# lehy/ocaml-hnsw

Measured on AMD Instinct MI355X. Metric: queries/sec at recall@10>=0.95, SIFT1M d=128 ef=128 k=10, higher is better.
Workload: dtype u8

## Files before the change

### include/hnsw_mi355x.h

```cpp
#ifndef HNSW_MI355X_H
#define HNSW_MI355X_H

#include <stdint.h>

#ifdef __cplusplus
extern "C" {
#endif

#define HNSW_ABI_VERSION 3

typedef struct hnsw_index hnsw_index;

enum {
    HNSW_OK = 0,
    HNSW_ERR_BAD_ARG = -1,
    HNSW_ERR_EMPTY_INDEX = -2,
    HNSW_ERR_DEGREE_OVERFLOW = -3,
    HNSW_ERR_NO_DEVICE = -4,
    HNSW_ERR_HIP = -5,
    HNSW_ERR_OOM = -6,
    HNSW_ERR_UNSUPPORTED = -7
};

enum { HNSW_METRIC_L2 = 0,
// ... 53 lines not shown
    int32_t row_format;
} hnsw_index_info;

int32_t hnsw_abi_version(void);
const char *hnsw_last_error(void);
int32_t hnsw_device_count(int32_t *count);

int32_t hnsw_index_create(const hnsw_index_desc *desc, int32_t device, hnsw_index **out);
int32_t hnsw_index_destroy(hnsw_index *idx);
int32_t hnsw_index_get_info(const hnsw_index *idx, hnsw_index_info *info);
int32_t hnsw_index_set_option(hnsw_index *idx, const char *name, int64_t value);
int32_t hnsw_index_row_bytes(const hnsw_index *idx, int64_t *row_bytes);
int32_t hnsw_index_sq8_params(const hnsw_index *idx, float *lo, float *scale);
int32_t hnsw_index_sq8_codes(const hnsw_index *idx, uint8_t *out);
int32_t hnsw_index_kernel_times(hnsw_index *idx, double *search_ms, double *prepass_ms, int32_t *calls);

int32_t hnsw_search_batch(hnsw_index *idx, const float *queries, int64_t nq, int64_t q_stride,
                          const hnsw_search_params *params, int32_t *out_ids, float *out_dist,
                          uint32_t *out_ndist, uint32_t *out_nhops);

int32_t hnsw_host_register(void *p, int64_t bytes);
int32_t hnsw_host_unregister(void *p);
int32_t hnsw_host_alloc(void **out, int64_t bytes);
int32_t hnsw_host_free(void *p);

int32_t hnsw_search_batch_device(hnsw_index *idx, const float *d_queries, int64_t nq,
                                 int64_t q_stride, const hnsw_search_params *params,
                                 int32_t *d_ids, float *d_dist, uint32_t *d_ndist,
                                 uint32_t *d_nhops, uint32_t *d_status, void *stream);

// ... 129 lines not shown
```

### ocaml-hnsw_amd/__init__.py

```python
import ctypes as _C
import os as _os

import numpy as _np

_PKG_DIR = _os.path.dirname(_os.path.abspath(__file__)) if "__file__" in globals() and \
    _os.path.basename(_os.path.dirname(_os.path.abspath(__file__))) == "ocaml-hnsw_amd" else \
    _os.path.join(_os.path.dirname(_os.path.abspath(__file__)), "ocaml-hnsw_amd")
LIB_PATH = _os.environ.get("HNSW_LIB_PATH") or _os.path.join(_PKG_DIR, "libhnsw_mi355x.so")

OK, ERR_BAD_ARG, ERR_EMPTY_INDEX, ERR_DEGREE_OVERFLOW = 0, -1, -2, -3
ERR_NO_DEVICE, ERR_HIP, ERR_OOM, ERR_UNSUPPORTED = -4, -5, -6, -7
METRIC_L2, METRIC_IP = 0, 1
FILL_OHNSW, FILL_BA = 0, 1
SEM_OHNSW, SEM_FUNCTOR, SEM_FUNCTOR_NEAREST_K = 0, 1, 2
ROWS_F32, ROWS_BYTES, ROWS_SPLIT, ROWS_HALF, ROWS_SQ8 = 0, 2, 3, 4, 5

ABI_VERSION = 3

_vp, _i32, _i64, _str, _f32 = _C.c_void_p, _C.c_int32, _C.c_int64, _C.c_char_p, _C.c_float
_ABI = {
    "hnsw_abi_version": (None, _i32),
    "hnsw_last_error": (None, _str),
    "hnsw_device_count": [_vp],
    "hnsw_index_create": [_vp, _i32, _vp],
# ... 27 lines not shown
    "hnsw_index_insert": [_vp, _vp, _i64, _i64, _vp],
    "hnsw_select_neighbours_batch": [_vp, _vp, _i64, _i64, _vp, _vp, _i32, _i32, _i32, _vp, _vp, _vp],
    "hnsw_index_layer_stats": [_vp, _i32, _vp],
    "hnsw_index_layer_isolated": [_vp, _i32, _vp, _i64, _vp],
    "hnsw_index_locality_codes": [_vp, _vp],
    "hnsw_index_visited_blocks": [_vp, _vp, _vp],
    "hnsw_index_prepare": [_vp, _vp],
    "hnsw_index_save": [_vp, _str],
    "hnsw_index_load": [_str, _i32, _vp],
    "hnsw_index_export_layer0": [_vp, _vp, _vp],
    "hnsw_index_export_upper_count": [_vp, _i32, _vp],
    "hnsw_index_export_upper": [_vp, _i32, _vp, _vp, _vp],
    "hnsw_search_layer_batch": [_vp, _i32, _vp, _i64, _i64, _vp, _i32, _vp, _vp, _vp, _vp, _vp, _vp],
    "hnsw_search_one_batch": [_vp, _i32, _vp, _i64, _i64, _vp, _vp, _vp],
    "hnsw_index_kernel_times": [_vp, _vp, _vp, _vp],
    "hnsw_search_submit": [_vp, _vp, _i64, _i64, _vp, _vp],
    "hnsw_search_wait": [_vp, _vp, _vp, _vp, _vp],
    "hnsw_multi_create": [_vp, _vp, _i32, _vp],
    "hnsw_multi_destroy": [_vp],
    "hnsw_multi_num_replicas": [_vp, _vp],
    "hnsw_multi_replica": [_vp, _i32, _vp],
    "hnsw_multi_search_batch": [_vp, _vp, _i64, _i64, _vp, _vp, _vp, _vp, _vp],
    "hnsw_multi_search_batch_device": [_vp, _vp, _i64, _i64, _vp, _vp, _vp],
    "hnsw_multi_copy_result": [_vp, _i32, _vp, _vp],
    "hnsw_multi_debug_counters": [_vp, _vp],
    "hnsw_host_register": [_vp, _i64],
    "hnsw_host_unregister": [_vp],
    "hnsw_host_alloc": [_vp, _i64],
    "hnsw_host_free": [_vp],
}
# ... 301 lines not shown
        return _np.float32(lo.value), _np.float32(s.value)

    def sq8_codes(self):
        out = _np.empty((self.info().n, self.d), _np.uint8)
        _check(load().hnsw_index_sq8_codes(self.handle, _ptr(out)))
        return out

    def filter(self, allow):
        return Filter(self, allow)

    def kernel_times(self):
        s_, p_, n_ = _C.c_double(0), _C.c_double(0), _C.c_int32(0)
        _check(load().hnsw_index_kernel_times(self.handle, _C.byref(s_), _C.byref(p_), _C.byref(n_)))
        return s_.value, p_.value, n_.value

    def release(self):
        if self._index is not None:
            load().hnsw_index_destroy(self._index)
            self._index = None

    def __del__(self):
        try:
            self.release()
        except Exception:
            pass


class _HostBlock:

    def __init__(self, shape, dtype):
# ... 453 lines not shown
```

### ocaml-hnsw_amd/build.py

```python
#!/usr/bin/env python3
import os
import subprocess
import sys

HERE = os.path.dirname(os.path.abspath(__file__))
CSRC = os.path.join(HERE, "csrc")
ROOT = os.path.dirname(HERE)
LIB = os.path.join(HERE, "libhnsw_mi355x.so")
SOURCES = ["hnsw_capi.hip", "hnsw_build.hip", "hnsw_layer_ops.hip", "hnsw_multi.hip", "hnsw_order.hip", "hnsw_rows8.hip",
           "hnsw_rows_split.hip", "hnsw_rows16.hip", "hnsw_rows_sq8.hip", "hnsw_locality.hip", "hnsw_scan.hip", "hnsw_rerank.hip", "hnsw_filter.hip",
           "hnsw_range.hip"]
VARIANT_SOURCE = "hnsw_search_variants.hip"
VARIANTS = [(m, s, f) for m in (0, 1) for s in (0, 1) for f in (0, 1, 2, 3, 4)]
DEPS = SOURCES + [VARIANT_SOURCE, "hnsw_device.hip.h", "hnsw_hop_asm.hip.h", "hnsw_hop_loop.inc", "hnsw_hop_slots.inc", "hnsw_hop_instances.inc", "hnsw_scan_slab.inc", "hnsw_build_device.hip.h", "hnsw_internal.h",
        os.path.join(ROOT, "include", "hnsw_mi355x.h")]


def _hipcc():
    for c in (os.environ.get("HIPCC"), "/opt/rocm/bin/hipcc", "hipcc"):
        if c and (os.path.isabs(c) and os.path.exists(c) or not os.path.isabs(c)):
            return c
    return "hipcc"


def up_to_date():
    if not os.path.exists(LIB):
        return False
    t = os.path.getmtime(LIB)
    for d in DEPS + [os.path.abspath(__file__)]:
# ... 88 lines not shown
```

### ocaml-hnsw_amd/csrc/hnsw_capi.hip

```cpp
#include "hnsw_internal.h"

#include <mutex>

using hnsw_dev::IndexView;
using hnsw_dev::SearchArgs;
using namespace hnsw_host;

__global__ void __launch_bounds__(64)
probe_queries_kernel(const IndexView iv, int64_t step, float *out) {
    const int64_t v = (int64_t)blockIdx.x * step;
    const int32_t nb = iv.nbr0[v * iv.S0];
    const int64_t u = nb >= 0 ? (int64_t)nb : v;
    for (int64_t i = threadIdx.x; i < iv.stride; i += 64)
        out[(int64_t)blockIdx.x * iv.stride + i] = 0.5f * (iv.X[v * iv.stride + i] + iv.X[u * iv.stride + i]);
}

__global__ void __launch_bounds__(1024)
flagged_list_kernel(const uint32_t *status, int64_t nq, int32_t *map, int32_t cap) {
    __shared__ int32_t count;
    if (threadIdx.x == 0) count = 0;
    for (int i = threadIdx.x; i < cap; i += blockDim.x) map[i] = -1;
    __syncthreads();
    for (int64_t q = threadIdx.x; q < nq; q += blockDim.x)
        if (status[q] & 1u) { const int at = atomicAdd(&count, 1); if (at < cap) map[at] = (int32_t)q; }
// ... 377 lines not shown
    if (nq == 0) return HNSW_OK;
    if (!buffers) return fail(HNSW_ERR_BAD_ARG, "null buffer");
    if (q_stride < idx->iv.d) return fail(HNSW_ERR_BAD_ARG, "q_stride < d");
    return HNSW_OK;
}

int launch_rerun(hnsw_index *idx, const hnsw_search_params &p, const KnnBatch &b, const int32_t *qmap, int64_t c, uint32_t *slab,
                 int32_t cap, hipStream_t st) {
    const KnnShape sh = knn_shape(idx, p.ef, p.semantics);
    SearchArgs a = knn_args(p, b, knn_vt_bits(idx, sh), knn_blk_bits(idx, sh));
    a.nq = c; a.qmap = qmap; a.q_limit = b.nq; a.ovf_g = slab; a.ovf_gcap = cap;
    a.any_flag = nullptr;
    return launch_search_args(idx, sh, a, st);
}

int knn_search(hnsw_index *idx, const hnsw_search_params *caller_params, const KnnBatch &caller_b, hipStream_t st, float *d_stage,
               RefineBufs *walk, bool raw_walk) {
    int rc = check_batch(idx, caller_params, caller_b.nq, caller_b.q_stride, caller_b.Q && caller_b.ids && caller_b.dist);
    if (rc || caller_b.nq == 0) return rc;
    HIP_TRY(hipSetDevice(idx->device));
    const int refine_c = raw_walk ? 0 : refine_count(idx, caller_params);
    hnsw_search_params walk_params = *caller_params;
    KnnBatch b = caller_b;
    if (refine_c > 0) {
        walk_params.k = refine_c;
        if ((rc = refine_walk(caller_b, refine_c, walk ? *walk : idx->refine_scratch, &b))) return rc;
    }
    const hnsw_search_params *params = &walk_params;
    const KnnShape sh = knn_shape(idx, params->ef, params->semantics);
    void *block = nullptr;
    Event *ev = nullptr;
    if (idx->time_kernels && idx->tev_used + 3 <= 3 * 4096) {
        while (idx->tev.size() < idx->tev_used + 3) {
            Event e;
            HIP_TRY(hipEventCreate(&e.h));
            idx->tev.push_back(std::move(e));
        }
        ev = &idx->tev[idx->tev_used];
        HIP_TRY(hipEventRecord(ev[0], st));
    }
    const bool sq8 = idx->info.row_format == HNSW_ROWS_SQ8;
    const float *rerank_Q = nullptr;
    if (sq8) {
        if ((rc = sq8_walk_queries(idx, walk ? *walk : idx->refine_scratch, &b, true, d_stage, st))) return rc;
        rerank_Q = d_stage ? d_stage : caller_b.Q;
        d_stage = nullptr;
    }
    SearchArgs a = knn_args(*params, b, knn_vt_bits(idx, sh), knn_blk_bits(idx, sh));
    const int mode = idx->order_mode;
    if (mode != 0 && (mode == 1 || 2 * b.nq > resident_queries(idx, sh).queries)) {
        rc = order_longest_first(idx, b.Q, b.nq, b.q_stride, d_stage, st, &block, &a.qmap, &a.pre_entry, &a.pre_key, &a.pre_nd, &a.pre_layer);
        if (rc) return rc;
// ... 51 lines not shown
}

hipError_t knn_download(const KnnBatch &b, int k, int32_t *ids, float *dist, uint32_t *nd, uint32_t *nh, hipStream_t st) {
    const size_t rbytes = (size_t)b.nq * k * 4, cbytes = (size_t)b.nq * 4;
    hipError_t e = hipSuccess;
    if (ids) e = hipMemcpyAsync(ids, b.ids, rbytes, hipMemcpyDeviceToHost, st);
    if (dist && e == hipSuccess) e = hipMemcpyAsync(dist, b.dist, rbytes, hipMemcpyDeviceToHost, st);
    if (nd && e == hipSuccess) e = hipMemcpyAsync(nd, b.nd, cbytes, hipMemcpyDeviceToHost, st);
    if (nh && e == hipSuccess) e = hipMemcpyAsync(nh, b.nh, cbytes, hipMemcpyDeviceToHost, st);
    return e;
}

int ensure_host_call_state(hnsw_index *idx) {
    if (!idx->hs[0]) HIP_TRY(hipStreamCreateWithFlags(&idx->hs[0].h, hipStreamNonBlocking));
    if (!idx->hFlag) {
        HIP_TRY(idx->hFlag.alloc(64, hipHostMallocMapped));
        HIP_TRY(hipHostGetDevicePointer((void **)&idx->hFlagDev, idx->hFlag, 0));
    }
    return HNSW_OK;
}

int HostInput::resolve(const void *p, size_t n, DevBuf &stage) {
    bytes = n; from = nullptr;
    if ((dev = registered_device_address(p, n))) return HNSW_OK;
    const int rc = stage.ensure(n);
    dev = stage.p; from = p;
    return rc;
}
int HostInput::upload(hipStream_t st) const {
    if (from) HIP_TRY(hipMemcpyAsync(const_cast<void *>(dev), from, bytes, hipMemcpyHostToDevice, st));
    return HNSW_OK;
}
// ... 24 lines not shown
        if (out_nd) znd = (uint32_t *)(s + 3 * SMALL_BLOCK);
        if (out_nh) znh = (uint32_t *)(s + 4 * SMALL_BLOCK);
    }
    k = k_;
    b = idx->scratch.batch(nq, q_stride, k);
    b.Q = (const float *)q.dev;
    if (zi) b.ids = zi, b.dist = zd;
    if (znd) b.nd = znd;
    if (znh) b.nh = znh;
    ids = zi && !small ? nullptr : out_ids; dist = zi && !small ? nullptr : out_dist;
    nd = znd && !small ? nullptr : out_nd; nh = znh && !small ? nullptr : out_nh;
    if (q_in_place) *q_in_place = !q.from;
    return q.upload(idx->hs[0]);
}

int HostCall::finish(hnsw_index *idx, const char *what, hipStream_t st) {
    const hipError_t ed = small ? hipSuccess : knn_download(b, k, ids, dist, nd, nh, st), es = st ? hipStreamSynchronize(st) : hipDeviceSynchronize();
    if (ed != hipSuccess) return hip_fail(ed, "result download");
    if (es != hipSuccess) return fail(HNSW_ERR_HIP, "%s failed: %s", what, hipGetErrorString(es));
    if (small) {
        const size_t rbytes = (size_t)b.nq * k * 4, cbytes = (size_t)b.nq * 4;
        memcpy(ids, idx->hSmall + SMALL_BLOCK, rbytes); memcpy(dist, idx->hSmall + 2 * SMALL_BLOCK, rbytes);
        if (nd) memcpy(nd, idx->hSmall + 3 * SMALL_BLOCK, cbytes);
        if (nh) memcpy(nh, idx->hSmall + 4 * SMALL_BLOCK, cbytes);
    }
    return HNSW_OK;
}

int trial_search(hnsw_index *idx, hnsw_search_params p) {
    int rc = ensure_host_call_state(idx);
    if (rc) return rc;
    DevBuf out;
// ... 295 lines not shown
                HIP_TRY(hipSetDevice(idx->device));
                HIP_TRY(hipDeviceSynchronize());
                idx->tables.Xq.release();
            }
            idx->sq8_on = false;
        }
        bind_view(idx);
        idx->forget_shapes();
        return HNSW_OK;
    }
    if (!strcmp(name, "refine")) {
        if (value < -1 || value > 1024) return fail(HNSW_ERR_BAD_ARG, "refine=%lld: 0 (off), 1..1024 candidates or -1 (all of W)", (long long)value);
        idx->refine = (int)value;
        return HNSW_OK;
    }
    if (!strcmp(name, "time_kernels")) { idx->time_kernels = value != 0; return HNSW_OK; }
    if (!strcmp(name, "visited_blocks")) {
        idx->blk_mode = value < 0 ? -1 : (value ? 1 : 0);
        idx->forget_shapes();
        return HNSW_OK;
    }
    if (!strcmp(name, "device_fallback_slab_bytes")) {
        HIP_TRY(hipSetDevice(idx->device));
        HIP_TRY(hipDeviceSynchronize());
        idx->dFbSlab.release(); idx->dFbMap.release(); idx->fb_queries = 0;
        if (value <= 0) return HNSW_OK;
        const int64_t per_query = std::max<int64_t>(idx->iv.n, 1) * 4;
        const int64_t q = std::min<int64_t>(value / per_query, 65536);
        if (q < 1) return fail(HNSW_ERR_BAD_ARG, "device_fallback_slab_bytes=%lld holds no query: one needs 4 n = %lld bytes", (long long)value, (long long)per_query);
        int rc;
        DevBuf slab, map;
// ... 21 lines not shown
    for (size_t i = 0; i < n; ++i) {
        float a = 0, b = 0;
        HIP_TRY(hipEventSynchronize(idx->tev[3 * i + 2]));
        HIP_TRY(hipEventElapsedTime(&a, idx->tev[3 * i], idx->tev[3 * i + 1]));
        HIP_TRY(hipEventElapsedTime(&b, idx->tev[3 * i + 1], idx->tev[3 * i + 2]));
        if (idx->tev_ordered[i]) p += a;
        s += b;
    }
    idx->tev_used = 0;
    if (search_ms) *search_ms = n ? s / (double)n : 0.0;
    if (prepass_ms) *prepass_ms = n ? p / (double)n : 0.0;
    if (calls) *calls = (int32_t)n;
    return HNSW_OK;
}

int32_t hnsw_search_batch(hnsw_index *idx, const float *queries, int64_t nq, int64_t q_stride,
                          const hnsw_search_params *params, int32_t *out_ids, float *out_dist,
                          uint32_t *out_ndist, uint32_t *out_nhops) {
    int rc = check_batch(idx, params, nq, q_stride, queries && out_ids && out_dist);
    if (rc || nq == 0) return rc;
    HIP_TRY(hipSetDevice(idx->device));
    HostCall c;
    bool q_in_place = false;
    if ((rc = c.begin(idx, queries, nq, q_stride, params->k, out_ids, out_dist, out_ndist, out_nhops, true, &q_in_place))) return rc;
    hipStream_t st = idx->hs[0];
    c.b.any_flag = idx->hFlagDev;
    *(volatile uint32_t *)idx->hFlag = 0;
    rc = knn_search(idx, params, c.b, st, q_in_place ? (float *)idx->scratch.q.p : nullptr);
    if (rc) { (void)hipStreamSynchronize(st); return rc; }
    if ((rc = c.finish(idx, "search", st))) return rc;
    if (*(volatile uint32_t *)idx->hFlag & 1u) {
        if ((rc = knn_repair(idx, params, c.b, nullptr))) return rc;
        return c.finish(idx, "result download", nullptr);
    }
    return HNSW_OK;
}

int32_t hnsw_search_batch_h2d(hnsw_index *idx, const float *queries, int64_t nq, int64_t q_stride,
                              const hnsw_search_params *params, int32_t *d_ids, float *d_dist,
                              uint32_t *d_ndist, uint32_t *d_nhops, uint32_t *d_status, void *stream) {
    int rc = check_batch(idx, params, nq, q_stride, queries && d_ids && d_dist);
    if (rc || nq == 0) return rc;
    HIP_TRY(hipSetDevice(idx->device));
    const size_t qbytes = query_bytes(nq, q_stride, idx->iv.d);
    if ((rc = idx->scratch.q.ensure(qbytes))) return rc;
    hipStream_t st = (hipStream_t)stream;
// ... 196 lines not shown
```

### ocaml-hnsw_amd/csrc/hnsw_device.hip.h

```cpp
#pragma once

#include <hip/hip_runtime.h>
#include <stdint.h>

namespace hnsw_dev {

constexpr uint32_t KEY_INF = 0xFFFFFFFFu;

struct IndexView {
    const float *X;
    int64_t stride;
    int64_t n;
    int32_t d;
    int32_t nchunks;
    const int32_t *nbr0;
    int32_t S0;
    int32_t SU;
    const int32_t *nbrU;
    int64_t rowsU;
    const int32_t *upper_off;
    const uint8_t *upper_lvl;
    const int2 *upper_ref;
    int32_t max_layer;
    int32_t entry_point;
    int32_t id_base;
    union { const uint8_t *X8; const uint2 *Xh; };
    int32_t stride8;
    const float *Xm;
    const float *tail0;
    int32_t stride_m;
    int32_t main_chunks;
    int32_t tail_chunks;
    const int32_t *lcode;
    const int32_t *lcode0;
};

struct SearchArgs {
    const float *Q;
    int64_t q_stride;
    int64_t nq;
    int32_t ef, k, fill;
    int32_t sem;
    int32_t vt_bits;
    int32_t blk_bits;
    int32_t lds_pad;
    int32_t *out_ids;
    float *out_dist;
    uint32_t *out_ndist, *out_nhops, *out_status;
    const int32_t *qmap;
    int64_t q_limit;
// ... 1029 lines not shown
        }
        cx.qint = ballot(ok) == ~0ull;
        cx.q2 = reduce16_i32((int32_t)sq);
    }
}
template <int NCH>
__device__ __forceinline__ void load_row(float4 (&qv)[NCH], const IndexView &iv, int node, int l16) {
    const float4 *row = reinterpret_cast<const float4 *>(iv.X) + (int64_t)node * (iv.stride >> 2);
#pragma unroll
    for (int i = 0; i < NCH; ++i) {
        const int c = i * 16 + l16;
        qv[i] = (c < iv.nchunks) ? row[c] : make_float4(0.f, 0.f, 0.f, 0.f);
    }
}

constexpr int search_min_waves(int NCH, int NSLOT, int METRIC, int ROWS) {
    return (NCH <= 2 && NSLOT <= 2 && METRIC == 0 && ROWS == 1) ? 7 : (NCH == 2 && NSLOT <= 4 && METRIC == 0 && ROWS == 2) ? 8 : 1;
}
template <int NCH, int RB, int NSLOT, int METRIC, int SEMF, int ROWS, int BLK = 0>
__global__ void __launch_bounds__(64, search_min_waves(NCH, NSLOT, METRIC, ROWS))
hnsw_search_kernel(const IndexView iv, const SearchArgs a) {
    extern __shared__ uint32_t lds[];
    const int lane = threadIdx.x;
    if ((int64_t)blockIdx.x >= a.nq) return;
    const int64_t q = a.qmap ? a.qmap[blockIdx.x] : (int64_t)blockIdx.x;
    if (a.q_limit && (q < 0 || q >= a.q_limit)) return;
    WaveCtx cx = make_ctx(lds, a.vt_bits, lane, BLK ? a.blk_bits : 0);
    if (a.ovf_g) { cx.ovf.g = a.ovf_g + (int64_t)blockIdx.x * a.ovf_gcap; cx.ovf.gcap = a.ovf_gcap; }
    if constexpr (NSLOT >= 3 || (NSLOT == 2 && ROWS != 2)) visited_three_ways(cx, iv.n);
    if ((int)blockIdx.x < a.prio_head || (int)blockIdx.x >= a.prio_tail) __builtin_amdgcn_s_setprio(3);
// ... 33 lines not shown
    search_layer<NCH, RB, NSLOT, METRIC, SEMF, ROWS, BLK>(iv, qv, 0, w, a.ef | (a.lds_pad << 16), cx, n_dist, n_hops, status);
#else
    search_layer<NCH, RB, NSLOT, METRIC, SEMF, ROWS, BLK>(iv, qv, 0, w, a.ef, cx, n_dist, n_hops, status);
#endif

    int wbase = NSLOT * 64 - a.ef;
    if (a.sem == 2) { const int cnt = wlist_count(w); wbase += cnt > a.k ? cnt - a.k : 0; }
#pragma unroll
    for (int s = 0; s < NSLOT; ++s) {
        const int idx = s * 64 + lane - wbase;
        if (idx >= 0 && idx < a.k) {
            int32_t oid = -1;
            float od = a.fill == 0 ? __uint_as_float(0x7FC00000u) : __uint_as_float(0x7F800000u);
            const uint32_t hi = w.hi[s];
            if (hi < DUMMY_HI) { oid = (int32_t)key_id(w.lo[s]) + iv.id_base; od = key_to_dist<METRIC>(hi); }
            a.out_ids[q * a.k + idx] = oid;
            a.out_dist[q * a.k + idx] = od;
        }
    }
    if (lane == 0) {
#ifdef HNSW_TIMING
        if (a.out_ndist) a.out_ndist[q] = (uint32_t)t_start__;
        if (a.out_nhops) a.out_nhops[q] = (uint32_t)wall_clock64();
#else
        if (a.out_ndist) a.out_ndist[q] = n_dist;
        if (a.out_nhops) a.out_nhops[q] = n_hops;
#endif
        if (a.out_status) a.out_status[q] = status;
#ifndef HNSW_PHASE_TIMING
        if ((status & 1u) && a.any_flag) *reinterpret_cast<volatile uint32_t *>(a.any_flag) = 1u;
#endif
    }
}

template <int NCH, int RB, int METRIC, int ROWS = -1>
__global__ void __launch_bounds__(64)
hnsw_descent_kernel(const IndexView iv, const float *Q, int64_t q_stride, int64_t nq, int32_t to_layer,
                    int32_t *out_entry, uint32_t *out_key, uint32_t *out_nd,
                    uint32_t *out_sortkey, int32_t *out_index, float *stage) {
    extern __shared__ uint32_t lds[];
    const int lane = threadIdx.x;
    const int64_t q = blockIdx.x;
    if (q >= nq) return;
    WaveCtx cx = make_ctx(lds, 4, lane);
    float4 qv[NCH];
    load_query<NCH>(qv, Q + q * q_stride, iv.d, cx.l16);
// ... 103 lines not shown
```

### ocaml-hnsw_amd/csrc/hnsw_internal.h

```cpp
#pragma once
#include "../../include/hnsw_mi355x.h"
#include "hnsw_device.hip.h"

#include <algorithm>
#include <cmath>
#include <cstdarg>
#include <cstdio>
#include <cstdlib>
#include <cstring>
#include <memory>
#include <string>
#include <type_traits>
#include <vector>

namespace hnsw_host {


constexpr int RB_NCH2 = 4;
constexpr int rows_in_flight(int nch, bool compact = false) {
    return nch == 1 ? 8 : nch == 2 ? RB_NCH2 : nch == 4 ? (compact ? 4 : 2) : nch == 8 ? (compact ? 2 : 1) : 1;
}
constexpr bool has_odd_nslot(int nch) { return nch == 2 || nch == 4; }

template <int V> using Int = std::integral_constant<int, V>;
// ... 103 lines not shown
    const float *Q;
    int64_t nq, q_stride;
    int32_t *ids;
    float *dist;
    uint32_t *nd, *nh, *st, *any_flag;
};

inline size_t query_bytes(int64_t nq, int64_t q_stride, int d) { return ((size_t)(nq - 1) * q_stride + d) * sizeof(float); }

struct BatchBufs {
    DevBuf q, ids, dist, nd, nh, st, flag, scan;
    KnnBatch batch(int64_t nq, int64_t q_stride, int k, int64_t row0 = 0) const {
        return {(const float *)q.p, nq, q_stride, (int32_t *)ids.p + row0 * k, (float *)dist.p + row0 * k,
                (uint32_t *)nd.p, (uint32_t *)nh.p, (uint32_t *)st.p, (uint32_t *)flag.p};
    }
    int ensure(int64_t nq, size_t qbytes, int k) {
        int rc;
        if ((rc = q.ensure(qbytes)) || (rc = ids.ensure((size_t)nq * k * 4)) || (rc = dist.ensure((size_t)nq * k * 4)) ||
            (rc = nd.ensure((size_t)nq * 4)) || (rc = nh.ensure((size_t)nq * 4)) || (rc = st.ensure((size_t)nq * 4)) || (rc = flag.ensure(16)))
            return rc;
        return HNSW_OK;
    }
    void release() { for (DevBuf *b : {&q, &ids, &dist, &nd, &nh, &st, &flag, &scan}) b->release(); }
};

struct RefineBufs {
    DevBuf ids, dist, nd, qt;
    int ensure(int64_t nq, int c) {
        int rc;
        if ((rc = ids.ensure((size_t)nq * c * 4)) || (rc = dist.ensure((size_t)nq * c * 4)) || (rc = nd.ensure((size_t)nq * 4))) return rc;
        return HNSW_OK;
    }
};

struct FilterBufs {
    DevBuf wids, wdist, wnd, wnh, wst;
// ... 65 lines not shown
    int lcode_state = 0;
    int blk_mode = -1;
    struct ShapeChoice {
        int blk = -1;
        int vt_bits = 0;
        int per_cu = -1;
        size_t lds = 0;
    } shape[hnsw_host::SLOT_CLASSES][2];
    void forget_shapes(bool keep_visited = false) {
        for (auto &c : shape) for (ShapeChoice &s : c) s = ShapeChoice{keep_visited ? s.blk : -1};
    }
    int cus = 0;
    hnsw_host::BatchBufs scratch;
    hnsw_host::Pinned<uint32_t> hFlag;
    uint32_t *hFlagDev = nullptr;
    hnsw_host::Pinned<char> hSmall;
    char *hSmallDev = nullptr;
    hnsw_host::DevBuf dFbSlab, dFbMap;
    int64_t fb_queries = 0;
    hnsw_host::Stream hs[4];
    std::vector<hnsw_request *> free_requests;
    std::vector<std::unique_ptr<hnsw_request>> all_requests;
    int live_requests = 0, next_stream = 0;
    bool time_kernels = false;
    std::vector<hnsw_host::Event> tev;
    size_t tev_used = 0;
    std::vector<char> tev_ordered;
    struct OrderScratch { hipStream_t st; hnsw_host::Table block; };
    std::vector<OrderScratch> order_scratch;
    int order_mode = -1;
    int vt_bits_override = 0;
    int lds_pad = -1;
    int scan_slabs = 0;
    std::vector<std::pair<int, int>> prepared;
    bool byte_rows_off = false, split_rows_off = false, split_rows_freed = false;
    bool half_rows_on = false;
    int refine = 0;
    hnsw_host::RefineBufs refine_scratch;
    bool sq8_on = false;
    float sq8_lo = 0.0f, sq8_scale = 1.0f;
    hnsw_host::FilterBufs filter_scratch;
    hnsw_host::RangeBufs range_scratch;
// ... 55 lines not shown
struct HostInput {
    const void *dev = nullptr, *from = nullptr;
    size_t bytes = 0;
    int resolve(const void *p, size_t n, DevBuf &stage);
    int upload(hipStream_t st) const;
};
struct HostCall {
    KnnBatch b{};
    int k = 0;
    bool small = false;
    int32_t *ids = nullptr;
    float *dist = nullptr;
    uint32_t *nd = nullptr, *nh = nullptr;
    int begin(::hnsw_index *idx, const float *queries, int64_t nq, int64_t q_stride, int k, int32_t *out_ids, float *out_dist,
              uint32_t *out_nd, uint32_t *out_nh, bool allow_small, bool *q_in_place = nullptr);
    int finish(::hnsw_index *idx, const char *what, hipStream_t st);
};

inline int search_vt_bits(const hnsw_index *idx, int ef) {
    int b = idx->vt_bits_override;
    if (b <= 0) {
        b = ef <= 256 ? 11 : 12;
    }
    b = std::max(4, std::min(16, b));
    while (b < 16 && ((int64_t)0xFFFF << (b - 1)) < idx->iv.n) ++b;
    return b;
}

template <class Launch>
int rerun_overflowed(hnsw_index *idx, int64_t nq, const uint32_t *d_status, Launch &&launch) {
    std::vector<uint32_t> st((size_t)nq);
// ... 20 lines not shown
```

### ocaml-hnsw_amd/csrc/hnsw_multi.hip

```cpp
#include "hnsw_internal.h"

#include <dlfcn.h>
#include <rccl/rccl.h>

using namespace hnsw_host;

namespace {

struct RcclApi {
    void *lib = nullptr;
    ncclResult_t (*CommInitAll)(ncclComm_t *, int, const int *) = nullptr;
    ncclResult_t (*CommDestroy)(ncclComm_t) = nullptr;
    ncclResult_t (*CommAbort)(ncclComm_t) = nullptr;
    ncclResult_t (*AllGather)(const void *, void *, size_t, ncclDataType_t, ncclComm_t, hipStream_t) = nullptr;
    ncclResult_t (*Broadcast)(const void *, void *, size_t, ncclDataType_t, int, ncclComm_t, hipStream_t) = nullptr;
    ncclResult_t (*GroupStart)() = nullptr;
    ncclResult_t (*GroupEnd)() = nullptr;
    const char *(*GetErrorString)(ncclResult_t) = nullptr;
};

int load_rccl(RcclApi &api) {
    if (api.lib) return HNSW_OK;
    void *h = nullptr;
    for (const char *name : {"librccl.so.1", "librccl.so", "/opt/rocm/lib/librccl.so.1"}) {
// ... 84 lines not shown
}

int search_and_gather(hnsw_multi *m, const float *queries, int64_t nq, int64_t q_stride, const hnsw_search_params *params,
                      uint32_t *out_ndist, uint32_t *out_nhops) {
    const int G = (int)m->replicas.size();
    const int k = params->k;
    int rc;
    if ((rc = ensure_streams(m)) || (rc = ensure_comms(m))) return rc;
    const int d = m->replicas[0]->iv.d;
    const size_t full = (size_t)nq * k;
    for (int g = 0; g < G; ++g) {
        const int64_t lo = shard_lo(nq, g, G), hi = shard_lo(nq, g + 1, G);
        hnsw_index *idx = m->replicas[(size_t)g];
        BatchBufs &b = m->buf[(size_t)g];
        HIP_TRY(hipSetDevice(m->devices[(size_t)g]));
        if ((rc = b.ids.ensure(std::max<size_t>(full, 1) * 4)) || (rc = b.dist.ensure(std::max<size_t>(full, 1) * 4)) || (rc = b.flag.ensure(16)))
            return rc;
        m->hFlags[g] = 0;
        if (hi <= lo) continue;
        const int64_t ns = hi - lo;
        const size_t qbytes = query_bytes(ns, q_stride, d);
        if ((rc = b.q.ensure(qbytes)) || (rc = b.nd.ensure((size_t)ns * 4)) || (rc = b.nh.ensure((size_t)ns * 4)) || (rc = b.st.ensure((size_t)ns * 4)))
            return rc;
        hipStream_t st = m->streams[(size_t)g];
        const KnnBatch shard = b.batch(ns, q_stride, k, lo);
        HIP_TRY(hipMemsetAsync(shard.any_flag, 0, 4, st));
        HIP_TRY(hipMemcpyAsync(b.q.p, queries + lo * q_stride, qbytes, hipMemcpyHostToDevice, st));
        if ((rc = knn_search(idx, params, shard, st))) return rc;
        HIP_TRY(hipMemcpyAsync(&m->hFlags[g], shard.any_flag, 4, hipMemcpyDeviceToHost, st));
    }
    auto exchange = [&](int only_shard) -> int {
// ... 195 lines not shown
```

### ocaml-hnsw_amd/csrc/hnsw_order.hip

```cpp
#include "hnsw_internal.h"

#include <hipcub/hipcub.hpp>

using hnsw_dev::IndexView;
using namespace hnsw_host;

namespace {
constexpr int ORDER_BUCKETS = 2048;
constexpr int ORDER_THREADS = 1024;
template <int PER>
__global__ void __launch_bounds__(ORDER_THREADS)
order_bucket_kernel(const uint32_t *sortkey, int32_t n, int32_t *order) {
    __shared__ uint32_t cnt[ORDER_BUCKETS];
    __shared__ uint32_t red_min[ORDER_THREADS / 64], red_max[ORDER_THREADS / 64];
    __shared__ uint32_t part[ORDER_THREADS];
    const int t = threadIdx.x;
    uint32_t keys[PER > 0 ? PER : 1];
    uint32_t lo = 0xFFFFFFFFu, hi = 0u;
    if (PER > 0) {
#pragma unroll
        for (int j = 0; j < PER; ++j) { const int i = t + j * ORDER_THREADS; keys[j] = sortkey[i < n ? i : 0]; }
#pragma unroll
        for (int j = 0; j < PER; ++j) if (t + j * ORDER_THREADS < n) { lo = keys[j] < lo ? keys[j] : lo; hi = keys[j] > hi ? keys[j] : hi; }
    } else {
// ... 70 lines not shown
    uint32_t *key = d_scratch, *nd = d_scratch + nq, *sortkey = d_scratch + 2 * nq;
    int32_t *index = (int32_t *)(d_scratch + 3 * nq);
    const int rows = idx->info.row_format == HNSW_ROWS_BYTES ? HNSW_ROWS_BYTES : HNSW_ROWS_F32;
    const hipError_t e = launch_descent(idx, rows, d_queries, q_stride, nq, to_layer, d_entry, key, nd, sortkey, index, nullptr, st);
    if (e != hipSuccess) return fail(HNSW_ERR_HIP, "descent launch failed: %s", hipGetErrorString(e));
    return HNSW_OK;
}

int order_longest_first(::hnsw_index *idx, const float *d_queries, int64_t nq, int64_t q_stride, float *d_stage, hipStream_t st,
                        void **block, const int32_t **qmap, const int32_t **pre_entry, const uint32_t **pre_key,
                        const uint32_t **pre_nd, int32_t *pre_layer) {
    const int32_t to_layer = 1;
    *pre_layer = to_layer;
    *block = nullptr;
    const size_t n = (size_t)nq, slot = (n * 4 + 255) & ~(size_t)255;
    size_t temp_bytes = 0;
    if (hipcub::DeviceRadixSort::SortPairs(nullptr, temp_bytes, (const uint32_t *)nullptr, (uint32_t *)nullptr,
                                           (const int32_t *)nullptr, (int32_t *)nullptr, (int)nq, 0, 32, st) != hipSuccess)
        return fail(HNSW_ERR_HIP, "radix sort sizing failed");
    temp_bytes = (temp_bytes + 255) & ~(size_t)255;
    const size_t need = 7 * slot + temp_bytes;
    hnsw_index::OrderScratch *sc = nullptr;
    for (auto &o : idx->order_scratch) if (o.st == st) sc = &o;
    if (!sc) { idx->order_scratch.push_back({st, {}}); sc = &idx->order_scratch.back(); }
    if (sc->block.bytes < need) {
        if (sc->block.p) HIP_TRY(hipStreamSynchronize(st));
        const size_t grow = need + need / 4;
        const hipError_t me = sc->block.alloc(grow);
        if (me != hipSuccess) return fail(me == hipErrorOutOfMemory ? HNSW_ERR_OOM : HNSW_ERR_HIP, "hipMalloc(%zu) for the ordering pre-pass failed", grow);
    }
    char *base = (char *)sc->block.p;
    hipError_t e;
    int32_t *entry = (int32_t *)(base + 0 * slot);
    uint32_t *key = (uint32_t *)(base + 1 * slot), *nd = (uint32_t *)(base + 2 * slot);
    uint32_t *sortkey = (uint32_t *)(base + 3 * slot), *sorted = (uint32_t *)(base + 4 * slot);
    int32_t *index = (int32_t *)(base + 5 * slot), *order = (int32_t *)(base + 6 * slot);
    void *temp = base + 7 * slot;
    e = launch_descent(idx, idx->info.row_format, d_queries, q_stride, nq, to_layer, entry, key, nd, sortkey, index, d_stage, st);
    if (e == hipSuccess) {
        if (nq <= 16 * ORDER_THREADS) {
            static_assert(ORDER_BUCKETS == 2 * ORDER_THREADS, "two counters per thread in the scan");
            hipLaunchKernelGGL(order_bucket_kernel<16>, dim3(1), dim3(ORDER_THREADS), 0, st, (const uint32_t *)sortkey, (int32_t)nq, order);
            e = hipGetLastError();
        } else {
            e = hipcub::DeviceRadixSort::SortPairs(temp, temp_bytes, (const uint32_t *)sortkey, sorted, (const int32_t *)index, order, (int)nq, 0, 32, st);
        }
    }
    if (e != hipSuccess) return fail(HNSW_ERR_HIP, "ordering pre-pass failed: %s", hipGetErrorString(e));
    *block = base; *qmap = order; *pre_entry = entry; *pre_key = key; *pre_nd = nd;
    return HNSW_OK;
}

}
```

### ocaml-hnsw_amd/ocaml/hnsw_mi355x.ml

```ocaml
open Ctypes
open Foreign

let lib = Dl.dlopen ~filename:"libhnsw_mi355x.so" ~flags:[ Dl.RTLD_NOW ]

type layer_desc
let layer_desc : layer_desc structure typ = structure "hnsw_layer_desc"
let ld_n_nodes = field layer_desc "n_nodes" int64_t
let ld_nodes = field layer_desc "nodes" (ptr int64_t)
let ld_deg = field layer_desc "deg" (ptr int32_t)
let ld_nbr = field layer_desc "nbr" (ptr int32_t)
let () = seal layer_desc

type index_desc
let index_desc : index_desc structure typ = structure "hnsw_index_desc"
let d_vectors = field index_desc "vectors" (ptr float)
let d_n = field index_desc "n" int64_t
let d_d = field index_desc "d" int32_t
let d_row_stride = field index_desc "row_stride" int64_t
let d_metric = field index_desc "metric" int32_t
let d_id_base = field index_desc "id_base" int32_t
let d_max_degree0 = field index_desc "max_degree0" int32_t
let d_max_degree = field index_desc "max_degree" int32_t
let d_max_layer = field index_desc "max_layer" int32_t
let d_entry_point = field index_desc "entry_point" int64_t
(* ... 32 lines not shown *)
let hnsw_search_one_batch =
  foreign ~from:lib ~release_runtime_lock:true "hnsw_search_one_batch"
    (index @-> int32_t @-> ptr float @-> int64_t @-> int64_t @-> ptr int64_t @-> ptr int64_t
     @-> ptr float @-> returning int32_t)
let hnsw_index_set_option =
  foreign ~from:lib "hnsw_index_set_option" (index @-> string @-> int64_t @-> returning int32_t)
let hnsw_index_row_bytes =
  foreign ~from:lib "hnsw_index_row_bytes" (index @-> ptr int64_t @-> returning int32_t)
let hnsw_index_sq8_params =
  foreign ~from:lib "hnsw_index_sq8_params" (index @-> ptr float @-> ptr float @-> returning int32_t)
let hnsw_index_sq8_codes =
  foreign ~from:lib ~release_runtime_lock:true "hnsw_index_sq8_codes" (index @-> ptr void @-> returning int32_t)
let hnsw_index_kernel_times =
  foreign ~from:lib ~release_runtime_lock:true "hnsw_index_kernel_times"
    (index @-> ptr double @-> ptr double @-> ptr int32_t @-> returning int32_t)
type request = unit ptr
let request : request typ = ptr void
let hnsw_search_submit =
  foreign ~from:lib ~release_runtime_lock:true "hnsw_search_submit"
    (index @-> ptr float @-> int64_t @-> int64_t @-> ptr search_params @-> ptr request @-> returning int32_t)
let hnsw_search_wait =
  foreign ~from:lib ~release_runtime_lock:true "hnsw_search_wait"
    (request @-> ptr int32_t @-> ptr float @-> ptr uint32_t @-> ptr uint32_t @-> returning int32_t)
type multi = unit ptr
let multi : multi typ = ptr void
let hnsw_multi_create =
  foreign ~from:lib ~release_runtime_lock:true "hnsw_multi_create"
    (ptr index_desc @-> ptr int32_t @-> int32_t @-> ptr multi @-> returning int32_t)
let hnsw_multi_destroy = foreign ~from:lib "hnsw_multi_destroy" (multi @-> returning int32_t)
let hnsw_multi_search_batch =
(* ... 782 lines not shown *)
```

Baseline: 22.10 million.

## Signal search completion via device counter and host-polled mapped flag

Adds a device-side completion counter: each search block atomically increments it, and the last block writes a sequence value into a host-mapped pinned flag word. For calls whose results land directly in host-visible memory, the host spins on that word for a bounded budget instead of calling hipStreamSynchronize, falling back to a stream sync on timeout. Output stores become system-scope atomics so results are visible before the flag. This removes sync latency from small batches, at the cost of CPU spinning, extra atomics per block, and more complex error and reset handling. The radix-sort temp sizing is also skipped when the bucket path is used.

```diff
diff --git a/include/hnsw_mi355x.h b/include/hnsw_mi355x.h
--- a/include/hnsw_mi355x.h
+++ b/include/hnsw_mi355x.h
@@ -91,6 +91,7 @@
 int32_t hnsw_index_sq8_params(const hnsw_index *idx, float *lo, float *scale);
 int32_t hnsw_index_sq8_codes(const hnsw_index *idx, uint8_t *out);
 int32_t hnsw_index_kernel_times(hnsw_index *idx, double *search_ms, double *prepass_ms, int32_t *calls);
+int32_t hnsw_index_completion_counts(const hnsw_index *idx, int64_t *polled, int64_t *synchronised);
 
 int32_t hnsw_search_batch(hnsw_index *idx, const float *queries, int64_t nq, int64_t q_stride,
                           const hnsw_search_params *params, int32_t *out_ids, float *out_dist,
diff --git a/ocaml-hnsw_amd/__init__.py b/ocaml-hnsw_amd/__init__.py
--- a/ocaml-hnsw_amd/__init__.py
+++ b/ocaml-hnsw_amd/__init__.py
@@ -65,6 +65,7 @@
     "hnsw_search_layer_batch": [_vp, _i32, _vp, _i64, _i64, _vp, _i32, _vp, _vp, _vp, _vp, _vp, _vp],
     "hnsw_search_one_batch": [_vp, _i32, _vp, _i64, _i64, _vp, _vp, _vp],
     "hnsw_index_kernel_times": [_vp, _vp, _vp, _vp],
+    "hnsw_index_completion_counts": [_vp, _vp, _vp],
     "hnsw_search_submit": [_vp, _vp, _i64, _i64, _vp, _vp],
     "hnsw_search_wait": [_vp, _vp, _vp, _vp, _vp],
     "hnsw_multi_create": [_vp, _vp, _i32, _vp],
@@ -396,6 +397,11 @@
         _check(load().hnsw_index_kernel_times(self.handle, _C.byref(s_), _C.byref(p_), _C.byref(n_)))
         return s_.value, p_.value, n_.value
 
+    def completion_counts(self):
+        a, b = _C.c_int64(0), _C.c_int64(0)
+        _check(load().hnsw_index_completion_counts(self.handle, _C.byref(a), _C.byref(b)))
+        return a.value, b.value
+
     def release(self):
         if self._index is not None:
             load().hnsw_index_destroy(self._index)
diff --git a/ocaml-hnsw_amd/build.py b/ocaml-hnsw_amd/build.py
--- a/ocaml-hnsw_amd/build.py
+++ b/ocaml-hnsw_amd/build.py
@@ -13,6 +13,7 @@
 VARIANT_SOURCE = "hnsw_search_variants.hip"
 VARIANTS = [(m, s, f) for m in (0, 1) for s in (0, 1) for f in (0, 1, 2, 3, 4)]
 DEPS = SOURCES + [VARIANT_SOURCE, "hnsw_device.hip.h", "hnsw_hop_asm.hip.h", "hnsw_hop_loop.inc", "hnsw_hop_slots.inc", "hnsw_hop_instances.inc", "hnsw_scan_slab.inc", "hnsw_build_device.hip.h", "hnsw_internal.h",
+        os.path.join(HERE, "host", "hnsw_wait.hpp"),
         os.path.join(ROOT, "include", "hnsw_mi355x.h")]
 
 
diff --git a/ocaml-hnsw_amd/csrc/hnsw_capi.hip b/ocaml-hnsw_amd/csrc/hnsw_capi.hip
--- a/ocaml-hnsw_amd/csrc/hnsw_capi.hip
+++ b/ocaml-hnsw_amd/csrc/hnsw_capi.hip
@@ -415,6 +415,17 @@
     return launch_search_args(idx, sh, a, st);
 }
 
+int reserve_timing_events(hnsw_index *idx, size_t need) {
+    if (idx->tev.size() >= need) return HNSW_OK;
+    const size_t want = std::min<size_t>(3 * 4096, std::max(need, std::max<size_t>(2 * idx->tev.size(), 3 * 32)));
+    while (idx->tev.size() < want) {
+        Event e;
+        HIP_TRY(hipEventCreate(&e.h));
+        idx->tev.push_back(std::move(e));
+    }
+    return HNSW_OK;
+}
+
 int knn_search(hnsw_index *idx, const hnsw_search_params *caller_params, const KnnBatch &caller_b, hipStream_t st, float *d_stage,
                RefineBufs *walk, bool raw_walk) {
     int rc = check_batch(idx, caller_params, caller_b.nq, caller_b.q_stride, caller_b.Q && caller_b.ids && caller_b.dist);
@@ -432,11 +443,7 @@
     void *block = nullptr;
     Event *ev = nullptr;
     if (idx->time_kernels && idx->tev_used + 3 <= 3 * 4096) {
-        while (idx->tev.size() < idx->tev_used + 3) {
-            Event e;
-            HIP_TRY(hipEventCreate(&e.h));
-            idx->tev.push_back(std::move(e));
-        }
+        if ((rc = reserve_timing_events(idx, idx->tev_used + 3))) return rc;
         ev = &idx->tev[idx->tev_used];
         HIP_TRY(hipEventRecord(ev[0], st));
     }
@@ -518,8 +525,16 @@
 int ensure_host_call_state(hnsw_index *idx) {
     if (!idx->hs[0]) HIP_TRY(hipStreamCreateWithFlags(&idx->hs[0].h, hipStreamNonBlocking));
     if (!idx->hFlag) {
+        static_assert(sizeof(hnsw_dev::FlagBlock) <= 64, "the handle's flag block");
         HIP_TRY(idx->hFlag.alloc(64, hipHostMallocMapped));
         HIP_TRY(hipHostGetDevicePointer((void **)&idx->hFlagDev, idx->hFlag, 0));
+        memset(idx->hFlag, 0, 64);
+    }
+    if (!idx->dDone.p) {
+        int rc = idx->dDone.ensure(16);
+        if (rc) return rc;
+        const hipError_t e = hipMemset(idx->dDone.p, 0, 16);
+        if (e != hipSuccess) { idx->dDone.release(); return hip_fail(e, "completion counter"); }
     }
     return HNSW_OK;
 }
@@ -574,8 +589,12 @@
     return q.upload(idx->hs[0]);
 }
 
-int HostCall::finish(hnsw_index *idx, const char *what, hipStream_t st) {
-    const hipError_t ed = small ? hipSuccess : knn_download(b, k, ids, dist, nd, nh, st), es = st ? hipStreamSynchronize(st) : hipDeviceSynchronize();
+int HostCall::finish(hnsw_index *idx, const char *what, hipStream_t st, uint32_t poll_value) {
+    const hipError_t ed = small || poll_value ? hipSuccess : knn_download(b, k, ids, dist, nd, nh, st);
+    bool fell_back = false;
+    const hipError_t es = poll_value ? wait_word(idx->hFlag + 1, poll_value, COMPLETION_SPIN, [&] { fell_back = true; return hipStreamSynchronize(st); })
+                                     : st ? hipStreamSynchronize(st) : hipDeviceSynchronize();
+    ++(poll_value && !fell_back ? idx->polled_calls : idx->synced_calls);
     if (ed != hipSuccess) return hip_fail(ed, "result download");
     if (es != hipSuccess) return fail(HNSW_ERR_HIP, "%s failed: %s", what, hipGetErrorString(es));
     if (small) {
@@ -901,7 +920,12 @@
         idx->refine = (int)value;
         return HNSW_OK;
     }
-    if (!strcmp(name, "time_kernels")) { idx->time_kernels = value != 0; return HNSW_OK; }
+    if (!strcmp(name, "time_kernels")) {
+        idx->time_kernels = value != 0;
+        if (value != 0) { HIP_TRY(hipSetDevice(idx->device)); return reserve_timing_events(idx, 1); }
+        return HNSW_OK;
+    }
+    if (!strcmp(name, "poll_completion")) { idx->poll_completion = value != 0; return HNSW_OK; }
     if (!strcmp(name, "visited_blocks")) {
         idx->blk_mode = value < 0 ? -1 : (value ? 1 : 0);
         idx->forget_shapes();
@@ -953,6 +977,13 @@
     return HNSW_OK;
 }
 
+int32_t hnsw_index_completion_counts(const hnsw_index *idx, int64_t *polled, int64_t *synchronised) {
+    if (!idx) return fail(HNSW_ERR_BAD_ARG, "null index");
+    if (polled) *polled = idx->polled_calls;
+    if (synchronised) *synchronised = idx->synced_calls;
+    return HNSW_OK;
+}
+
 int32_t hnsw_search_batch(hnsw_index *idx, const float *queries, int64_t nq, int64_t q_stride,
                           const hnsw_search_params *params, int32_t *out_ids, float *out_dist,
                           uint32_t *out_ndist, uint32_t *out_nhops) {
@@ -965,10 +996,32 @@
     hipStream_t st = idx->hs[0];
     c.b.any_flag = idx->hFlagDev;
     *(volatile uint32_t *)idx->hFlag = 0;
+    uint32_t poll = 0;
+    if (idx->poll_completion && refine_count(idx, params) == 0 && idx->info.row_format != HNSW_ROWS_SQ8 &&
+        (c.small || (!c.ids && !c.dist && !c.nd && !c.nh))) {
+        if (++idx->done_seq == 0) ++idx->done_seq;
+        poll = idx->done_seq;
+    }
+    hnsw_dev::FlagBlock *const fb = (hnsw_dev::FlagBlock *)(uint32_t *)idx->hFlag;
+    auto signalling = [&](bool on) {
+        fb->done_value = poll; fb->done_counter = (uint32_t *)idx->dDone.p;
+        *(volatile uint32_t *)&fb->done_target = on ? (uint32_t)nq : 0u;
+    };
+    if (poll) signalling(true);
     rc = knn_search(idx, params, c.b, st, q_in_place ? (float *)idx->scratch.q.p : nullptr);
-    if (rc) { (void)hipStreamSynchronize(st); return rc; }
-    if ((rc = c.finish(idx, "search", st))) return rc;
+    if (rc) {
+        (void)hipStreamSynchronize(st);
+        if (poll) { signalling(false); (void)hipMemset(idx->dDone.p, 0, 4); }
+        return rc;
+    }
+    rc = c.finish(idx, "search", st, poll);
+    if (poll) {
+        signalling(false);
+        if (*(volatile uint32_t *)&fb->done_word != poll) (void)hipMemset(idx->dDone.p, 0, 4);
+    }
+    if (rc) return rc;
     if (*(volatile uint32_t *)idx->hFlag & 1u) {
+        if (poll) HIP_TRY(hipStreamSynchronize(st));
         if ((rc = knn_repair(idx, params, c.b, nullptr))) return rc;
         return c.finish(idx, "result download", nullptr);
     }
diff --git a/ocaml-hnsw_amd/csrc/hnsw_device.hip.h b/ocaml-hnsw_amd/csrc/hnsw_device.hip.h
--- a/ocaml-hnsw_amd/csrc/hnsw_device.hip.h
+++ b/ocaml-hnsw_amd/csrc/hnsw_device.hip.h
@@ -1,6 +1,7 @@
 #pragma once
 
 #include <hip/hip_runtime.h>
+#include <stddef.h>
 #include <stdint.h>
 
 namespace hnsw_dev {
@@ -34,6 +35,17 @@
     const int32_t *lcode;
     const int32_t *lcode0;
 };
+
+struct FlagBlock {
+    uint32_t any_flag;
+    uint32_t done_word;
+    uint32_t pad[2];
+    uint32_t done_target;
+    uint32_t done_value;
+    uint32_t *done_counter;
+};
+constexpr int FLAG_WORDS = 8;
+static_assert(sizeof(FlagBlock) == FLAG_WORDS * 4 && offsetof(FlagBlock, done_target) == 16 && offsetof(FlagBlock, done_counter) == 24, "FlagBlock");
 
 struct SearchArgs {
     const float *Q;
@@ -1093,6 +1105,23 @@
     }
 }
 
+__device__ __forceinline__ void search_block_done(uint32_t *any_flag) {
+    if (any_flag == nullptr) return;
+    typedef const __attribute__((address_space(4))) unsigned long long *k64;
+    const k64 desc = (k64)(reinterpret_cast<const unsigned long long *>(any_flag) + 2);
+    const unsigned long long tv = desc[0], cp = desc[1];
+    const uint32_t target = (uint32_t)tv, value = (uint32_t)(tv >> 32);
+    if (target == 0) return;
+    uint32_t *const counter = reinterpret_cast<uint32_t *>(cp);
+    asm volatile("s_waitcnt vmcnt(0)" ::: "memory");
+    const uint32_t before = __hip_atomic_fetch_add(counter, 1u, __ATOMIC_RELAXED, __HIP_MEMORY_SCOPE_AGENT);
+    if (before == target - 1u) {
+        __hip_atomic_store(counter, 0u, __ATOMIC_RELAXED, __HIP_MEMORY_SCOPE_AGENT);
+        __hip_atomic_store(any_flag + 1, value, __ATOMIC_RELEASE, __HIP_MEMORY_SCOPE_SYSTEM);
+    }
+}
+template <class T> __device__ __forceinline__ void store_out(T *p, T v) { __hip_atomic_store(p, v, __ATOMIC_RELAXED, __HIP_MEMORY_SCOPE_SYSTEM); }
+
 constexpr int search_min_waves(int NCH, int NSLOT, int METRIC, int ROWS) {
     return (NCH <= 2 && NSLOT <= 2 && METRIC == 0 && ROWS == 1) ? 7 : (NCH == 2 && NSLOT <= 4 && METRIC == 0 && ROWS == 2) ? 8 : 1;
 }
@@ -1156,22 +1185,23 @@
             float od = a.fill == 0 ? __uint_as_float(0x7FC00000u) : __uint_as_float(0x7F800000u);
             const uint32_t hi = w.hi[s];
             if (hi < DUMMY_HI) { oid = (int32_t)key_id(w.lo[s]) + iv.id_base; od = key_to_dist<METRIC>(hi); }
-            a.out_ids[q * a.k + idx] = oid;
-            a.out_dist[q * a.k + idx] = od;
+            store_out(&a.out_ids[q * a.k + idx], oid);
+            store_out(&a.out_dist[q * a.k + idx], od);
         }
     }
     if (lane == 0) {
 #ifdef HNSW_TIMING
-        if (a.out_ndist) a.out_ndist[q] = (uint32_t)t_start__;
-        if (a.out_nhops) a.out_nhops[q] = (uint32_t)wall_clock64();
+        if (a.out_ndist) store_out(&a.out_ndist[q], (uint32_t)t_start__);
+        if (a.out_nhops) store_out(&a.out_nhops[q], (uint32_t)wall_clock64());
 #else
-        if (a.out_ndist) a.out_ndist[q] = n_dist;
-        if (a.out_nhops) a.out_nhops[q] = n_hops;
+        if (a.out_ndist) store_out(&a.out_ndist[q], n_dist);
+        if (a.out_nhops) store_out(&a.out_nhops[q], n_hops);
 #endif
         if (a.out_status) a.out_status[q] = status;
 #ifndef HNSW_PHASE_TIMING
-        if ((status & 1u) && a.any_flag) *reinterpret_cast<volatile uint32_t *>(a.any_flag) = 1u;
-#endif
+        if ((status & 1u) && a.any_flag) store_out(a.any_flag, 1u);
+#endif
+        search_block_done(a.any_flag);
     }
 }
 
diff --git a/ocaml-hnsw_amd/csrc/hnsw_internal.h b/ocaml-hnsw_amd/csrc/hnsw_internal.h
--- a/ocaml-hnsw_amd/csrc/hnsw_internal.h
+++ b/ocaml-hnsw_amd/csrc/hnsw_internal.h
@@ -1,6 +1,7 @@
 #pragma once
 #include "../../include/hnsw_mi355x.h"
 #include "hnsw_device.hip.h"
+#include "../host/hnsw_wait.hpp"
 
 #include <algorithm>
 #include <cmath>
@@ -141,12 +142,20 @@
         return {(const float *)q.p, nq, q_stride, (int32_t *)ids.p + row0 * k, (float *)dist.p + row0 * k,
                 (uint32_t *)nd.p, (uint32_t *)nh.p, (uint32_t *)st.p, (uint32_t *)flag.p};
     }
+    int ensure_flag() {
+        if (flag.p) return HNSW_OK;
+        const int rc = flag.ensure(sizeof(hnsw_dev::FlagBlock));
+        if (rc) return rc;
+        const hipError_t e = hipMemset(flag.p, 0, sizeof(hnsw_dev::FlagBlock));
+        if (e != hipSuccess) { flag.release(); return hip_fail(e, "flag block"); }
+        return HNSW_OK;
+    }
     int ensure(int64_t nq, size_t qbytes, int k) {
         int rc;
         if ((rc = q.ensure(qbytes)) || (rc = ids.ensure((size_t)nq * k * 4)) || (rc = dist.ensure((size_t)nq * k * 4)) ||
-            (rc = nd.ensure((size_t)nq * 4)) || (rc = nh.ensure((size_t)nq * 4)) || (rc = st.ensure((size_t)nq * 4)) || (rc = flag.ensure(16)))
+            (rc = nd.ensure((size_t)nq * 4)) || (rc = nh.ensure((size_t)nq * 4)) || (rc = st.ensure((size_t)nq * 4)))
             return rc;
-        return HNSW_OK;
+        return ensure_flag();
     }
     void release() { for (DevBuf *b : {&q, &ids, &dist, &nd, &nh, &st, &flag, &scan}) b->release(); }
 };
@@ -242,6 +251,9 @@
     hnsw_host::BatchBufs scratch;
     hnsw_host::Pinned<uint32_t> hFlag;
     uint32_t *hFlagDev = nullptr;
+    bool poll_completion = true;
+    hnsw_host::DevBuf dDone;
+    uint32_t done_seq = 0;
     hnsw_host::Pinned<char> hSmall;
     char *hSmallDev = nullptr;
     hnsw_host::DevBuf dFbSlab, dFbMap;
@@ -254,6 +266,7 @@
     std::vector<hnsw_host::Event> tev;
     size_t tev_used = 0;
     std::vector<char> tev_ordered;
+    int64_t polled_calls = 0, synced_calls = 0;
     struct OrderScratch { hipStream_t st; hnsw_host::Table block; };
     std::vector<OrderScratch> order_scratch;
     int order_mode = -1;
@@ -339,7 +352,7 @@
     uint32_t *nd = nullptr, *nh = nullptr;
     int begin(::hnsw_index *idx, const float *queries, int64_t nq, int64_t q_stride, int k, int32_t *out_ids, float *out_dist,
               uint32_t *out_nd, uint32_t *out_nh, bool allow_small, bool *q_in_place = nullptr);
-    int finish(::hnsw_index *idx, const char *what, hipStream_t st);
+    int finish(::hnsw_index *idx, const char *what, hipStream_t st, uint32_t poll_value = 0);
 };
 
 inline int search_vt_bits(const hnsw_index *idx, int ef) {
diff --git a/ocaml-hnsw_amd/csrc/hnsw_multi.hip b/ocaml-hnsw_amd/csrc/hnsw_multi.hip
--- a/ocaml-hnsw_amd/csrc/hnsw_multi.hip
+++ b/ocaml-hnsw_amd/csrc/hnsw_multi.hip
@@ -122,7 +122,7 @@
         hnsw_index *idx = m->replicas[(size_t)g];
         BatchBufs &b = m->buf[(size_t)g];
         HIP_TRY(hipSetDevice(m->devices[(size_t)g]));
-        if ((rc = b.ids.ensure(std::max<size_t>(full, 1) * 4)) || (rc = b.dist.ensure(std::max<size_t>(full, 1) * 4)) || (rc = b.flag.ensure(16)))
+        if ((rc = b.ids.ensure(std::max<size_t>(full, 1) * 4)) || (rc = b.dist.ensure(std::max<size_t>(full, 1) * 4)) || (rc = b.ensure_flag()))
             return rc;
         m->hFlags[g] = 0;
         if (hi <= lo) continue;
diff --git a/ocaml-hnsw_amd/csrc/hnsw_order.hip b/ocaml-hnsw_amd/csrc/hnsw_order.hip
--- a/ocaml-hnsw_amd/csrc/hnsw_order.hip
+++ b/ocaml-hnsw_amd/csrc/hnsw_order.hip
@@ -108,9 +108,10 @@
     *pre_layer = to_layer;
     *block = nullptr;
     const size_t n = (size_t)nq, slot = (n * 4 + 255) & ~(size_t)255;
+    const bool radix = nq > 16 * ORDER_THREADS;
     size_t temp_bytes = 0;
-    if (hipcub::DeviceRadixSort::SortPairs(nullptr, temp_bytes, (const uint32_t *)nullptr, (uint32_t *)nullptr,
-                                           (const int32_t *)nullptr, (int32_t *)nullptr, (int)nq, 0, 32, st) != hipSuccess)
+    if (radix && hipcub::DeviceRadixSort::SortPairs(nullptr, temp_bytes, (const uint32_t *)nullptr, (uint32_t *)nullptr,
+                                                    (const int32_t *)nullptr, (int32_t *)nullptr, (int)nq, 0, 32, st) != hipSuccess)
         return fail(HNSW_ERR_HIP, "radix sort sizing failed");
     temp_bytes = (temp_bytes + 255) & ~(size_t)255;
     const size_t need = 7 * slot + temp_bytes;
@@ -132,7 +133,7 @@
     void *temp = base + 7 * slot;
     e = launch_descent(idx, idx->info.row_format, d_queries, q_stride, nq, to_layer, entry, key, nd, sortkey, index, d_stage, st);
     if (e == hipSuccess) {
-        if (nq <= 16 * ORDER_THREADS) {
+        if (!radix) {
             static_assert(ORDER_BUCKETS == 2 * ORDER_THREADS, "two counters per thread in the scan");
             hipLaunchKernelGGL(order_bucket_kernel<16>, dim3(1), dim3(ORDER_THREADS), 0, st, (const uint32_t *)sortkey, (int32_t)nq, order);
             e = hipGetLastError();
diff --git a/ocaml-hnsw_amd/host/hnsw_wait.hpp b/ocaml-hnsw_amd/host/hnsw_wait.hpp
--- /dev/null
+++ b/ocaml-hnsw_amd/host/hnsw_wait.hpp
@@ -0,0 +1,38 @@
+#pragma once
+
+#include <chrono>
+#include <cstdint>
+
+#if defined(__x86_64__) || defined(__i386__)
+#include <immintrin.h>
+#endif
+
+namespace hnsw_host {
+
+inline void cpu_pause() {
+#if defined(__x86_64__) || defined(__i386__)
+    _mm_pause();
+#elif defined(__aarch64__)
+    __asm__ __volatile__("yield");
+#endif
+}
+
+struct SpinBudget { std::chrono::nanoseconds ns; };
+constexpr SpinBudget COMPLETION_SPIN{std::chrono::microseconds(2000)};
+
+template <class Fallback>
+inline auto wait_word(volatile const uint32_t *word, uint32_t want, SpinBudget budget, Fallback &&fallback)
+    -> decltype(fallback()) {
+    using clock = std::chrono::steady_clock;
+    const clock::time_point t_end = clock::now() + budget.ns;
+    for (;;) {
+        for (int i = 0; i < 64; ++i) {
+            if (__atomic_load_n(const_cast<const uint32_t *>(word), __ATOMIC_ACQUIRE) == want) return decltype(fallback())();
+            cpu_pause();
+        }
+        if (clock::now() >= t_end) break;
+    }
+    return fallback();
+}
+
+}
diff --git a/ocaml-hnsw_amd/ocaml/hnsw_mi355x.ml b/ocaml-hnsw_amd/ocaml/hnsw_mi355x.ml
--- a/ocaml-hnsw_amd/ocaml/hnsw_mi355x.ml
+++ b/ocaml-hnsw_amd/ocaml/hnsw_mi355x.ml
@@ -70,6 +70,8 @@
 let hnsw_index_kernel_times =
   foreign ~from:lib ~release_runtime_lock:true "hnsw_index_kernel_times"
     (index @-> ptr double @-> ptr double @-> ptr int32_t @-> returning int32_t)
+let hnsw_index_completion_counts =
+  foreign ~from:lib "hnsw_index_completion_counts" (index @-> ptr int64_t @-> ptr int64_t @-> returning int32_t)
 type request = unit ptr
 let request : request typ = ptr void
 let hnsw_search_submit =
```

Measured after the change: 22.29 million (median of 6 runs). No clear change (+0.9%).
